# tub-rip/MotionPriorCMax

Measured on AMD Instinct MI355X. Metric: Mevents/s through CMax loss fwd+bwd, DSEC 480x640, higher is better.
Workload: dtype f32; 1 GPU; C3: DSEC 480x640, 200k events/window, poly-k3, batch=14 per GPU (BASELINE configs[2]; the per-GPU shard of configs[4] = batch 112 on 8 GPUs); batch_per_gpu=14, events_layout=time, resident_batches_rotated=4, global_batch=14, num_bins=15, num_knn=32, parallelism=dp1, grad_allreduce_MB=0

## Files before the change

### motionpriorcmax_amd/csrc/diag/stamps.h

```cpp
#pragma once

#ifdef KNN_BK_STAMP
#define BK_STAMP_DECL __shared__ unsigned s_stp[8];
#define BK_STAMP(k) do { __builtin_amdgcn_s_waitcnt(0); if (threadIdx.x == 0) s_stp[k] = (unsigned)wall_clock64(); } while (0)
#define BK_STAMP_WRITE(ls_, tid_) do { BK_STAMP(7); __syncthreads(); \
        if ((tid_) < 8) (ls_).fail[1 + 100000 + 8 * blockIdx.x + (tid_)] = (tid_) == 0 ? (int)s_stp[0] : (int)(s_stp[tid_] - s_stp[0]); } while (0)
#else
#define BK_STAMP_DECL
#define BK_STAMP(k) do { } while (0)
#define BK_STAMP_WRITE(ls_, tid_) do { } while (0)
#endif

#if defined(KS_STAMP2) || defined(KS_STAMP0)
#ifdef KS_STAMP0
#define KS_STP_ON (MODE == 0)
#else
#define KS_STP_ON (FARK)
#endif
#define KS_STP_DECL unsigned long long stp_[8]; int nstp_ = 0;
#define KS_STP() do { if (KS_STP_ON && nstp_ < 8) { __builtin_amdgcn_s_waitcnt(0); stp_[nstp_++] = wall_clock64(); } } while (0)
#define KS_STP_WRITE(ls_, tid_, mine_, total_) do { if (KS_STP_ON) { __syncthreads(); KS_STP(); const int nmk_ = __syncthreads_count((mine_) ? 1 : 0); \
        if ((tid_) == 0) { int *dst_ = (ls_).fail + 1 + 200000 + 12 * (int)blockIdx.x; dst_[0] = (int)(stp_[0] & 0x7fffffffull); \
            for (int k_ = 1; k_ < 8; ++k_) dst_[k_] = (int)(stp_[k_] - stp_[0]); dst_[8] = (total_); dst_[9] = nmk_; } } } while (0)
#else
#define KS_STP_DECL
#define KS_STP() do { } while (0)
#define KS_STP_WRITE(ls_, tid_, mine_, total_) do { } while (0)
#endif

#ifdef KS_DEBUG_INBIN
#define KS_INBIN_STAT(knn_state_, BQ_, q_, inbin_, nsl_, iwd_, norm_) do { (knn_state_)[2 * (BQ_) + (q_)] = (float)(inbin_) + 100.f * (float)(nsl_); } while (0)
#else
#define KS_INBIN_STAT(knn_state_, BQ_, q_, inbin_, nsl_, iwd_, norm_) do { if (iwd_) (knn_state_)[2 * (BQ_) + (q_)] = (norm_); } while (0)
#endif

#ifdef KNN_BW_STAMP
#define KB_STAMP_PARAM , int *__restrict__ stamp
#define KB_STAMP_BEGIN const unsigned long long st0 = wall_clock64(); int st_slow = 0;
#define KB_STAMP_MID const unsigned long long st1 = wall_clock64();
#define KB_STAMP_SLOW st_slow = 1;
#define KB_STAMP_END(tid_, lblk_, RQ_, use_lds_, anytie_, total_) do { __syncthreads(); const bool anyslow_ = __syncthreads_or(st_slow) != 0; \
        if ((tid_) == 0) { const unsigned long long st2_ = wall_clock64(); stamp[4 * (lblk_) + 0] = (int)(st2_ - st0); stamp[4 * (lblk_) + 1] = (int)(st1 - st0); \
            stamp[4 * (lblk_) + 2] = (RQ_) | ((use_lds_) ? 0 : 256) | ((anytie_) ? 512 : 0) | (anyslow_ ? 1024 : 0); stamp[4 * (lblk_) + 3] = (total_); } } while (0)
#define KB_STAMP_ARG(ws_, L_) , (int *)((char *)(ws_) + (L_).off_knn_fail)
#else
#define KB_STAMP_PARAM
#define KB_STAMP_BEGIN
#define KB_STAMP_MID
#define KB_STAMP_SLOW
#define KB_STAMP_END(tid_, lblk_, RQ_, use_lds_, anytie_, total_) do { } while (0)
#define KB_STAMP_ARG(ws_, L_)
#endif

#ifdef EV_LA_STAMP
#define LA_STAMP_DECL __shared__ unsigned s_stp[8]; if (threadIdx.x < 8) s_stp[threadIdx.x] = (unsigned)wall_clock64();
#define LA_STAMP(k) do { __builtin_amdgcn_s_waitcnt(0); if (threadIdx.x == 0) s_stp[k] = (unsigned)wall_clock64(); } while (0)
#define LA_STAMP_WRITE(tid_, dst_, n_) do { LA_STAMP(6); __syncthreads(); if ((tid_) == 0) { unsigned *d_ = reinterpret_cast<unsigned *>(dst_); \
        for (int k_ = 0; k_ < 7; ++k_) d_[k_] = s_stp[k_] - s_stp[0]; d_[7] = (unsigned)(n_); d_[8] = s_stp[0]; } } while (0)
#else
#define LA_STAMP_DECL
#define LA_STAMP(k) do { } while (0)
#define LA_STAMP_WRITE(tid_, dst_, n_) do { } while (0)
#endif

#ifdef KT_TIMELINE
#define KT_T(k_) do { __builtin_amdgcn_s_waitcnt(0); if (threadIdx.x == 0) kt_[k_] = (int)(wall_clock64() & 0x7fffffffull); } while (0)
#define KT_DECL int kt_[6] = {0, 0, 0, 0, 0, 0};
#define KT_COUNT(k_, n_) do { kt_[k_] = (n_); } while (0)
#define KT_WRITE(ls_) do { if (threadIdx.x == 0) { int *d_ = (ls_).fail + 1 + 300000 + 8 * (int)blockIdx.x; for (int k_ = 0; k_ < 6; ++k_) d_[k_] = kt_[k_]; } } while (0)
#else
#define KT_T(k_) do { } while (0)
#define KT_DECL
#define KT_COUNT(k_, n_) do { } while (0)
#define KT_WRITE(ls_) do { } while (0)
#endif
```

### motionpriorcmax_amd/csrc/events.hip

```cpp
#include "common.h"
#include "ev_count_device.h"
#include "knn_device.h"
#include "bounds.h"
#include "diag/stamps.h"

struct EvParams {
    int B, M, Mp, nb, T, H, W, sp, hq, wq, P;
    unsigned flags;
};

struct Warped {
    float y, x, w;
    int lut;
    float fy, fx;
    int y0, x0;
    int it, iy, ix;
};

__device__ __forceinline__ EvParams make_params(const mpc_shape s) {
    EvParams p;
    p.B = s.B; p.M = s.M; p.Mp = s.Mp; p.nb = s.nb; p.T = s.T; p.H = s.H; p.W = s.W;
    p.sp = s.sp; p.hq = s.hq; p.wq = s.wq;
    p.P = (s.flags & MPC_F_POLARITY_SPLIT) ? 2 : 1;
    p.flags = s.flags;
// ... 22 lines not shown
        const float dt = fminf(fmaxf(fabsf(e[2] - t_ref), 0.f), 1.f);
        w = (1.f - dt) * w;
    }
    if (p.flags & MPC_F_MASK_BORDER) {
        if (y > (float)p.H || x > (float)p.W || y < 0.f || x < 0.f) w = 0.f;
    }
    o.y = y; o.x = x; o.w = w;
    const float y0f = floorf(y + 1e-6f), x0f = floorf(x + 1e-6f);
    o.fy = y - y0f;
    o.fx = x - x0f;
    o.y0 = (int)fminf(fmaxf(y0f, -4.f), (float)p.H + 4.f);
    o.x0 = (int)fminf(fmaxf(x0f, -4.f), (float)p.W + 4.f);
    return w != 0.f;
}

__device__ __forceinline__ bool warp_event(const EvParams &p, const float e[6], int b, int tr,
                                           const float *__restrict__ lut, float t_ref, Warped &o) {
    o.lut = -1;
    float2 f = make_float2(0.f, 0.f);
    if (!(p.flags & MPC_F_NO_WARP)) {
        warp_cell(p, e, b, tr, o);
        f = reinterpret_cast<const float2 *>(lut)[o.lut];
    }
    return warp_event_with(p, e, f, t_ref, o);
}

__device__ __forceinline__ void load_event(const float *__restrict__ events, size_t row, float e[6]) {
    const float2 *p = reinterpret_cast<const float2 *>(events + row * 6);
    const float2 a = p[0], b = p[1], c = p[2];
    e[0] = a.x; e[1] = a.y; e[2] = b.x; e[3] = b.y; e[4] = c.x; e[5] = c.y;
}

__global__ __launch_bounds__(256) void k_splat_fwd_atomic(const mpc_shape s,
                                                          const float *__restrict__ events,
                                                          const float *__restrict__ lut,
                                                          const float *__restrict__ t_ref,
                                                          float *__restrict__ iwe) {
    const EvParams p = make_params(s);
    const size_t total = (size_t)p.B * p.M;
    for (size_t row = (size_t)blockIdx.x * 256 + threadIdx.x; row < total; row += (size_t)gridDim.x * 256) {
        const int b = (int)(row / p.M), i = (int)(row - (size_t)b * p.M);
        float e[6];
        load_event(events, row, e);
        const int pol = (p.P == 2 && i >= p.Mp) ? 1 : 0;
        for (int tr = 0; tr < p.T; ++tr) {
            Warped o;
            const float tref = (p.flags & MPC_F_SCALE_BY_DT) ? t_ref[tr] : 0.f;
            if (!warp_event(p, e, b, tr, lut, tref, o)) continue;
            float *img = iwe + ((size_t)(b * p.T + tr) * p.P + pol) * p.H * p.W;
            const float w00 = (1.f - o.fy) * (1.f - o.fx) * o.w;
            const float w10 = o.fy * (1.f - o.fx) * o.w;
            const float w01 = (1.f - o.fy) * o.fx * o.w;
            const float w11 = o.fy * o.fx * o.w;
            const bool yin0 = o.y0 >= 0 && o.y0 < p.H, yin1 = o.y0 + 1 >= 0 && o.y0 + 1 < p.H;
            const bool xin0 = o.x0 >= 0 && o.x0 < p.W, xin1 = o.x0 + 1 >= 0 && o.x0 + 1 < p.W;
            if (yin0 && xin0) atomicAdd(img + (size_t)o.y0 * p.W + o.x0, w00);
            if (yin1 && xin0) atomicAdd(img + (size_t)(o.y0 + 1) * p.W + o.x0, w10);
            if (yin0 && xin1) atomicAdd(img + (size_t)o.y0 * p.W + o.x0 + 1, w01);
            if (yin1 && xin1) atomicAdd(img + (size_t)(o.y0 + 1) * p.W + o.x0 + 1, w11);
        }
    }
}

__device__ __forceinline__ void event_pos_grad(const EvParams &p, const Warped &o,
                                               const float *__restrict__ g , float &gy,
                                               float &gx) {
    const bool yin0 = o.y0 >= 0 && o.y0 < p.H, yin1 = o.y0 + 1 >= 0 && o.y0 + 1 < p.H;
    const bool xin0 = o.x0 >= 0 && o.x0 < p.W, xin1 = o.x0 + 1 >= 0 && o.x0 + 1 < p.W;
    const float g00 = (yin0 && xin0) ? g[(size_t)o.y0 * p.W + o.x0] : 0.f;
    const float g10 = (yin1 && xin0) ? g[(size_t)(o.y0 + 1) * p.W + o.x0] : 0.f;
    const float g01 = (yin0 && xin1) ? g[(size_t)o.y0 * p.W + o.x0 + 1] : 0.f;
    const float g11 = (yin1 && xin1) ? g[(size_t)(o.y0 + 1) * p.W + o.x0 + 1] : 0.f;
    gy = o.w * ((1.f - o.fx) * (g10 - g00) + o.fx * (g11 - g01));
    gx = o.w * ((1.f - o.fy) * (g01 - g00) + o.fy * (g11 - g10));
}

__global__ __launch_bounds__(256) void k_splat_bwd_atomic(const mpc_shape s,
                                                          const float *__restrict__ events,
                                                          const float *__restrict__ lut,
                                                          const float *__restrict__ t_ref,
                                                          const float *__restrict__ gimg,
                                                          const float *__restrict__ scal,
                                                          const float *__restrict__ grad_out,
                                                          float *__restrict__ glut) {
    const EvParams p = make_params(s);
    const float coef = scal[MPC_SCAL_GCOEF] * (grad_out ? grad_out[0] : 1.f);
    const size_t total = (size_t)p.B * p.M;
    for (size_t row = (size_t)blockIdx.x * 256 + threadIdx.x; row < total; row += (size_t)gridDim.x * 256) {
        const int b = (int)(row / p.M), i = (int)(row - (size_t)b * p.M);
        float e[6];
        load_event(events, row, e);
        const int pol = (p.P == 2 && i >= p.Mp) ? 1 : 0;
        for (int tr = 0; tr < p.T; ++tr) {
            Warped o;
            const float tref = (p.flags & MPC_F_SCALE_BY_DT) ? t_ref[tr] : 0.f;
            if (!warp_event(p, e, b, tr, lut, tref, o)) continue;
            const float *img = gimg + ((size_t)(b * p.T + tr) * p.P + pol) * p.H * p.W;
            float gy, gx;
            event_pos_grad(p, o, img, gy, gx);
            atomicAdd(glut + 2 * (size_t)o.lut, coef * gy);
            atomicAdd(glut + 2 * (size_t)o.lut + 1, coef * gx);
        }
    }
}

__global__ __launch_bounds__(256) void k_event_pos_grad(const mpc_shape s, const float *__restrict__ events,
                                                        const float *__restrict__ t_ref, const float *__restrict__ gimg,
                                                        const float *__restrict__ scal, const float *__restrict__ grad_out,
                                                        float2 *__restrict__ gpos) {
    const EvParams p = make_params(s);
    const float coef = scal[MPC_SCAL_GCOEF] * (grad_out ? grad_out[0] : 1.f);
    const float tref = (p.flags & MPC_F_SCALE_BY_DT) ? t_ref[0] : 0.f;
    const size_t total = (size_t)p.B * p.M;
    for (size_t row = (size_t)blockIdx.x * 256 + threadIdx.x; row < total; row += (size_t)gridDim.x * 256) {
        const int b = (int)(row / p.M), i = (int)(row - (size_t)b * p.M);
        float e[6];
        load_event(events, row, e);
        const int pol = (p.P == 2 && i >= p.Mp) ? 1 : 0;
        Warped o;
        float2 g = make_float2(0.f, 0.f);
        if (warp_event_with(p, e, make_float2(0.f, 0.f), tref, o)) {
            float gy, gx;
            event_pos_grad(p, o, gimg + ((size_t)b * p.P + pol) * p.H * p.W, gy, gx);
            g = make_float2(coef * gy, coef * gx);
        }
        gpos[row] = g;
    }
}

#define EV_MARKER 0x6d706331

struct BinLayout {
    int SR, NS, CSR, NCS, NF, NBk, fcap, bcap, P, exact;
    int *gcount;
    int *bcapcnt;
    float4 *frec, *brec;
};

struct __attribute__((packed, aligned(4))) rec3 { float y, x, w; };

__device__ __forceinline__ long long ev_to_fixed_small(float v) {
    return (long long)(int)(v * (float)(1 << MPC_FIX_SHIFT));
}

__device__ __forceinline__ int xcd_swizzle(int p, int n) {
    const int per = (n + 7) >> 3;
    return (p & 7) * per + (p >> 3);
}


__device__ __forceinline__ void ev_emit(const EvParams &p, const BinLayout &L, int b, int nf_loc, int lb, int slot,
                                        float4 rec) {
    if (lb < nf_loc) {
        const int g = (b * p.P + lb / L.NS) * L.NS + (lb % L.NS);
        MPC_EXPECT(g >= 0 && g < L.NF);
        reinterpret_cast<rec3 *>(L.frec)[(size_t)g * L.fcap + MPC_IDX(slot, L.fcap)] = rec3{rec.x, rec.y, rec.z};
    } else {
        const size_t base = L.exact ? (size_t)b : (size_t)(b * p.nb * L.NCS + (lb - nf_loc));
        MPC_EXPECT((long long)base < (L.exact ? (long long)p.B : (long long)L.NBk));
        L.brec[base * L.bcap + MPC_IDX(slot, L.bcap)] = rec;
    }
}

__global__ __launch_bounds__(256) void k_ev_bin(const mpc_shape s, const BinLayout L,
                                                const float *__restrict__ events,
                                                const float *__restrict__ lut,
                                                const float *__restrict__ t_ref, int want_bwd,
                                                const int *__restrict__ offsets) {
    extern __shared__ __align__(16) int s_cnt[];
    __shared__ int s_wsum[4];
    const EvParams p = make_params(s);
    const int chunks = (p.M + 256 * EV_PER_THREAD - 1) / (256 * EV_PER_THREAD);
    const int lblk = xcd_swizzle(blockIdx.x, chunks * p.B);
    if (lblk >= chunks * p.B) return;
    const int tid = threadIdx.x, b = lblk / chunks, chunk = lblk - b * chunks;
    int pad0 = p.M, pad1 = p.M, blk1 = p.M;
    if (offsets != nullptr) {
        const int nk1 = p.nb * L.NCS + 1;
        const int *ob = offsets + (size_t)b * 2 * nk1;
        blk1 = p.Mp;
        pad0 = min(max(ob[nk1 - 1], 0), blk1);
        pad1 = min(max(ob[2 * nk1 - 1], blk1), p.M);
        const int c0 = chunk * EV_PER_THREAD * 256, c1 = min(c0 + EV_PER_THREAD * 256, p.M);
        const bool all_pad = (c0 >= pad0 && c1 <= blk1) || c0 >= pad1;
        if (all_pad) return;
    }
    const int nf_loc = p.P * L.NS, nb_loc = want_bwd ? p.nb * L.NCS : 0, nloc = nf_loc + nb_loc;
    int *s_base = s_cnt + nloc;
    const int stage_off = ((3 * nloc + 1 + EV_STAGE / 2) + 3) & ~3;
    for (int i = tid; i < nloc; i += 256) s_cnt[i] = 0;
    __syncthreads();
    const float tref = (p.flags & MPC_F_SCALE_BY_DT) ? t_ref[0] : 0.f;
    const float inv_SR = 1.f / (float)L.SR, inv_CSR = 1.f / (float)L.CSR;

    float ry[EV_PER_THREAD], rx[EV_PER_THREAD], rw[EV_PER_THREAD];
    int f0[EV_PER_THREAD], f1[EV_PER_THREAD], bk[EV_PER_THREAD];
    int r0[EV_PER_THREAD], r1[EV_PER_THREAD], rb[EV_PER_THREAD];
    unsigned aux[EV_PER_THREAD];
    float ev[EV_PER_THREAD][6];
    Warped wo[EV_PER_THREAD];
    bool live[EV_PER_THREAD];
#pragma unroll
    for (int k = 0; k < EV_PER_THREAD; ++k) {
        const int i = (chunk * EV_PER_THREAD + k) * 256 + tid;
        load_event(events, (size_t)b * p.M + min(i, p.M - 1), ev[k]);
    }
#pragma unroll
    for (int k = 0; k < EV_PER_THREAD; ++k) {
        const int i = (chunk * EV_PER_THREAD + k) * 256 + tid;
        live[k] = warp_event(p, ev[k], b, 0, lut, tref, wo[k]) && (i < p.M) && !((i >= pad0 && i < blk1) || i >= pad1);
    }
#pragma unroll
    for (int k = 0; k < EV_PER_THREAD; ++k) {
        const int i = (chunk * EV_PER_THREAD + k) * 256 + tid;
        f0[k] = f1[k] = bk[k] = -1;
        r0[k] = r1[k] = rb[k] = 0;
        ry[k] = rx[k] = rw[k] = 0.f; aux[k] = 0u;
        if (!live[k]) continue;
        const Warped &o = wo[k];
        const bool xin = (o.x0 + 1 >= 0) && (o.x0 < p.W);
        const bool yin0 = o.y0 >= 0 && o.y0 < p.H, yin1 = o.y0 + 1 >= 0 && o.y0 + 1 < p.H;
        if (!xin || !(yin0 || yin1)) continue;
        const int pol = (p.P == 2 && i >= p.Mp) ? 1 : 0;
        ry[k] = o.y; rx[k] = o.x; rw[k] = o.w;
        const int s0 = yin0 ? (int)(((float)o.y0 + 0.5f) * inv_SR) : -1, s1 = yin1 ? (int)(((float)o.y0 + 1.5f) * inv_SR) : -1;
        if (s0 >= 0) { f0[k] = pol * L.NS + s0; r0[k] = atomicAdd(&s_cnt[MPC_IDX(f0[k], nf_loc)], 1); }
        if (s1 >= 0 && s1 != s0) { f1[k] = pol * L.NS + s1; r1[k] = atomicAdd(&s_cnt[MPC_IDX(f1[k], nf_loc)], 1); }
        if (want_bwd && o.lut >= 0) {
            const int cst = (int)(((float)o.iy + 0.5f) * inv_CSR);
            bk[k] = nf_loc + o.it * L.NCS + cst;
            rb[k] = atomicAdd(&s_cnt[MPC_IDX(bk[k], nloc)], 1);
            aux[k] = ((unsigned)pol << 31) | (unsigned)((o.iy - cst * L.CSR) * p.wq + o.ix);
        }
    }
    __syncthreads();
    for (int i = tid; i < nloc; i += 256) {
        const int c = s_cnt[i];
        int g;
        int first = 0;
        if (i < nf_loc) g = (b * p.P + i / L.NS) * L.NS + (i % L.NS);
        else { g = L.NF + b * p.nb * L.NCS + (i - nf_loc); if (L.exact) first = L.bcapcnt[L.NBk + b * p.nb * L.NCS + (i - nf_loc)]; }
        s_base[i] = (c > 0 ? atomicAdd(&L.gcount[MPC_IDX(g, L.NF + L.NBk)], c) : 0) + first;
    }
    int *s_loc = s_base + nloc;
    unsigned short *s_bid = reinterpret_cast<unsigned short *>(s_loc + nloc + 1);
    float4 *s_rec = reinterpret_cast<float4 *>(s_cnt + stage_off);
    {
        const int per = (nloc + 255) >> 8;
        const int i0 = min(tid * per, nloc), i1 = min(i0 + per, nloc);
        int local = 0;
        for (int i = i0; i < i1; ++i) local += s_cnt[i];
        int incl = local;
#pragma unroll
        for (int o = 1; o < 64; o <<= 1) { const int v = __shfl_up(incl, o, 64); if ((tid & 63) >= o) incl += v; }
        if ((tid & 63) == 63) s_wsum[tid >> 6] = incl;
        __syncthreads();
        int run = incl - local;
        for (int w = 0; w < (tid >> 6); ++w) run += s_wsum[w];
        for (int i = i0; i < i1; ++i) { s_loc[i] = run; run += s_cnt[i]; }
        if (tid == 255) s_loc[nloc] = run;
    }
    __syncthreads();
    const int total = s_loc[nloc];
#pragma unroll
    for (int k = 0; k < EV_PER_THREAD; ++k) {
        if (f0[k] >= 0 || f1[k] >= 0) {
            const int polf = (f0[k] >= 0 ? f0[k] : f1[k]) / L.NS;
            const float4 rec = make_float4(ry[k], rx[k], rw[k], __int_as_float(b * p.P + polf));
#pragma unroll
            for (int h = 0; h < 2; ++h) {
                const int lb = h ? f1[k] : f0[k];
                if (lb < 0) continue;
                const int at = s_loc[lb] + (h ? r1[k] : r0[k]);
                if (at < EV_STAGE) { s_rec[MPC_IDX(at, EV_STAGE)] = rec; s_bid[MPC_IDX(at, EV_STAGE)] = (unsigned short)lb; }
                else ev_emit(p, L, b, nf_loc, lb, s_base[lb] + (h ? r1[k] : r0[k]), rec);
            }
        }
        if (bk[k] >= 0) {
            const float4 rec = make_float4(ry[k], rx[k], rw[k], __uint_as_float(aux[k]));
            const int at = s_loc[bk[k]] + rb[k];
            if (at < EV_STAGE) { s_rec[MPC_IDX(at, EV_STAGE)] = rec; s_bid[MPC_IDX(at, EV_STAGE)] = (unsigned short)bk[k]; }
            else ev_emit(p, L, b, nf_loc, bk[k], s_base[bk[k]] + rb[k], rec);
        }
    }
    __syncthreads();
    for (int r = tid; r < min(total, EV_STAGE); r += 256) {
        const int lb = s_bid[r];
        ev_emit(p, L, b, nf_loc, lb, s_base[MPC_IDX(lb, nloc)] + (r - s_loc[lb]), s_rec[r]);
    }
    if (want_bwd && lblk == 0 && tid == 0) L.gcount[L.NF + L.NBk + 2] = EV_MARKER;
}

template <typename F>
__device__ __forceinline__ void record_taps(float y, float x, float w, int H, int W, int row0, int row1, F f) {
    const float y0f = floorf(y + 1e-6f), x0f = floorf(x + 1e-6f);
    const float fy = y - y0f, fx = x - x0f;
    const int y0 = (int)fminf(fmaxf(y0f, -4.f), (float)H + 4.f), x0 = (int)fminf(fmaxf(x0f, -4.f), (float)W + 4.f);
    const bool r0 = y0 >= row0 && y0 < row1, r1 = y0 + 1 >= row0 && y0 + 1 < row1;
    const bool c0 = x0 >= 0 && x0 < W, c1 = x0 + 1 >= 0 && x0 + 1 < W;
    if (r0 && c0) f(y0, x0, (1.f - fy) * (1.f - fx) * w);
    if (r1 && c0) f(y0 + 1, x0, fy * (1.f - fx) * w);
    if (r0 && c1) f(y0, x0 + 1, (1.f - fy) * fx * w);
    if (r1 && c1) f(y0 + 1, x0 + 1, fy * fx * w);
}

template <bool FIXED>
__global__ __launch_bounds__(1024) void k_iwe_accum(const BinLayout L, float *__restrict__ iwe, int H, int W) {
    extern __shared__ unsigned long long s_acc[];
    const int tid = threadIdx.x;
    const int g = blockIdx.x, img = g / L.NS, strip = g - img * L.NS;
    const int row0 = strip * L.SR, row1 = min(row0 + L.SR, H);
    const int npix = (row1 - row0) * W;
    const int n = L.gcount[g];
    const rec3 *rec = reinterpret_cast<const rec3 *>(L.frec) + (size_t)g * L.fcap;
    rec3 e[4];
#pragma unroll
    for (int u = 0; u < 4; ++u) e[u] = rec[MPC_IDX(min(tid + u * 1024, L.fcap - 1), L.fcap)];
    for (int i = tid; i < npix; i += 1024) s_acc[i] = 0ull;
    __syncthreads();
    for (int r0 = tid; r0 < n; r0 += 4 * 1024) {
        if (r0 != tid) {
#pragma unroll
            for (int u = 0; u < 4; ++u) e[u] = rec[min(r0 + u * 1024, n - 1)];
        }
#pragma unroll
        for (int u = 0; u < 4; ++u) {
            if (r0 + u * 1024 >= n) continue;
            if (fabsf(e[u].w) <= 1.5f)
                record_taps(e[u].y, e[u].x, e[u].w, H, W, row0, row1, [&](int yy, int xx, float v) {
                    atomicAdd(&s_acc[MPC_IDX((yy - row0) * W + xx, npix)], (unsigned long long)ev_to_fixed_small(v));
                });
            else
                record_taps(e[u].y, e[u].x, e[u].w, H, W, row0, row1, [&](int yy, int xx, float v) {
                    atomicAdd(&s_acc[MPC_IDX((yy - row0) * W + xx, npix)], (unsigned long long)mpc_to_fixed(v));
                });
        }
    }
    __syncthreads();
    if (FIXED) {
        long long *dst = reinterpret_cast<long long *>(iwe) + ((size_t)img * H + row0) * W;
        for (int i = tid; i < npix; i += 1024) dst[i] = (long long)s_acc[i];
    } else {
        float *dst = iwe + ((size_t)img * H + row0) * W;
        for (int i = tid; i < npix; i += 1024) dst[i] = mpc_from_fixed((long long)s_acc[i]);
    }
}

__global__ __launch_bounds__(256) void k_iwe_from_fixed(const long long *__restrict__ src, float *__restrict__ dst, size_t n) {
    for (size_t i = (size_t)blockIdx.x * 256 + threadIdx.x; i < n; i += (size_t)gridDim.x * 256) dst[i] = mpc_from_fixed(src[i]);
}

struct __attribute__((packed, aligned(4))) pair4 { float x, y; };

__device__ __forceinline__ void record_grad(float y, float x, float w, const float *__restrict__ g, int H, int W,
                                            float &gy, float &gx) {
    const float y0f = floorf(y + 1e-6f), x0f = floorf(x + 1e-6f);
    const float fy = y - y0f, fx = x - x0f;
    const int y0 = (int)fminf(fmaxf(y0f, -4.f), (float)H + 4.f), x0 = (int)fminf(fmaxf(x0f, -4.f), (float)W + 4.f);
    const bool r0 = y0 >= 0 && y0 < H, r1 = y0 + 1 >= 0 && y0 + 1 < H;
    const bool c0 = x0 >= 0 && x0 < W, c1 = x0 + 1 >= 0 && x0 + 1 < W;
    const int xa = min(max(x0, 0), W - 2);
    const int ya = min(max(y0, 0), H - 1), yb = min(max(y0 + 1, 0), H - 1);
    const pair4 a = *reinterpret_cast<const pair4 *>(g + MPC_IDX((size_t)ya * W + xa, (long long)H * W - 1));
    const pair4 b = *reinterpret_cast<const pair4 *>(g + MPC_IDX((size_t)yb * W + xa, (long long)H * W - 1));
    const bool lo = (xa == x0);
    const float g00 = (r0 && c0) ? (lo ? a.x : a.y) : 0.f;
    const float g01 = (r0 && c1) ? (lo ? a.y : a.x) : 0.f;
    const float g10 = (r1 && c0) ? (lo ? b.x : b.y) : 0.f;
    const float g11 = (r1 && c1) ? (lo ? b.y : b.x) : 0.f;
    gy = w * ((1.f - fx) * (g10 - g00) + fx * (g11 - g01));
    gx = w * ((1.f - fy) * (g01 - g00) + fy * (g11 - g10));
}

template <bool ORDERED>
__global__ __launch_bounds__(ORDERED ? EV_LUT_THREADS_ORD : EV_LUT_THREADS, ORDERED ? 1 : EV_LUT_MINWAVES) void k_lut_accum(const mpc_shape s, const BinLayout L,
                                                    const float *__restrict__ gimg,
                                                    const float *__restrict__ scal,
                                                    const float *__restrict__ grad_out,
                                                    float *__restrict__ glut,
                                                    const float *__restrict__ add_term,
                                                    const float *__restrict__ events, const float *__restrict__ lut,
                                                    const float *__restrict__ t_ref, const int *__restrict__ offsets,
                                                    const KnnReachJob job) {
    extern __shared__ unsigned long long s_acc[];
    LA_STAMP_DECL
    constexpr int NT = ORDERED ? EV_LUT_THREADS_ORD : EV_LUT_THREADS, NIF = ORDERED ? EV_LUT_INFLIGHT_ORD : EV_LUT_INFLIGHT;
    constexpr int APF = ORDERED ? 0 : EV_LUT_ADD_PF;
    const EvParams p = make_params(s);
    const int tid = threadIdx.x;
    const int lg = xcd_swizzle(blockIdx.x, L.NBk);
    if (lg >= L.NBk) return;
    const int b = lg / (L.NCS * p.nb), rem = lg - b * (L.NCS * p.nb);
    const int cst = rem / p.nb, it = rem - cst * p.nb;
    const int bt = b * p.nb + it;
    const int g = bt * L.NCS + cst;
    const int crow0 = cst * L.CSR, crow1 = min(crow0 + L.CSR, p.hq);
    const int ncell = (crow1 - crow0) * p.wq;
    const int NK = p.nb * L.NCS, key = it * L.NCS + cst;
    float4 e[NIF];
    float2 addv[APF > 0 ? APF : 1];
    int mark = 0, n = 0;
    float gcoef = 0.f, gout = 1.f;
    const float4 *rec = L.brec;
    int rcap = L.bcap;
    const float2 *add = add_term ? reinterpret_cast<const float2 *>(add_term) + ((size_t)bt * p.hq + crow0) * p.wq : nullptr;
    const bool spec = !ORDERED && !(p.flags & MPC_F_NO_BWD_RECORDS);
    if (!ORDERED) {
        mark = L.gcount[L.NF + L.NBk + 2];
        n = L.gcount[L.NF + g];
        int first = 0;
        if (L.exact) first = min(max(L.bcapcnt[L.NBk + (size_t)b * NK + key], 0), L.bcap - 1);
        rec = L.brec + (size_t)(L.exact ? b : g) * L.bcap + first;
        rcap = L.bcap - first;
        const float4 *src = spec ? rec : reinterpret_cast<const float4 *>(L.gcount);
        const int last = spec ? rcap - 1 : 0;
#pragma unroll
        for (int u = 0; u < NIF; ++u) e[u] = src[MPC_IDX(min(tid + u * NT, last), last + 1)];
        gcoef = scal[MPC_SCAL_GCOEF];
        if (grad_out) gout = grad_out[0];
        if (add && ncell > 0) {
#pragma unroll
            for (int k = 0; k < APF; ++k) addv[k] = add[MPC_IDX(min(tid + k * NT, ncell - 1), ncell)];
        }
    }
    if (job.on && cst == 0) {
        if (job.p.l1) knn_reach_slice<true>(job.p, job.tile_dkmax, job.reach, bt, job.gx, job.gy, job.bd, reinterpret_cast<float *>(s_acc));
        else knn_reach_slice<false>(job.p, job.tile_dkmax, job.reach, bt, job.gx, job.gy, job.bd, reinterpret_cast<float *>(s_acc));
        __syncthreads();
    }
    for (int i = tid; i < 2 * ncell; i += NT) s_acc[i] = 0ull;
    float2 *s_lut = reinterpret_cast<float2 *>(s_acc + 2 * ncell);
    if (ORDERED) {
        const float2 *src = reinterpret_cast<const float2 *>(lut) + ((size_t)(b * p.nb + it) * p.hq + crow0) * p.wq;
        for (int i = tid; i < ncell; i += NT) s_lut[i] = src[i];
    }
    __syncthreads();
    LA_STAMP(1);
    const bool valid = ORDERED || mark == EV_MARKER;
    int n_pos = 0, o_pos = 0, o_neg = 0;
    if (ORDERED) {
        const int *ob = offsets + (size_t)b * 2 * (NK + 1);
        o_pos = min(max(ob[key], 0), p.M); n_pos = min(max(ob[key + 1] - o_pos, 0), p.M - o_pos);
// ... 7 lines not shown
        const int pol = r >= n_pos ? 1 : 0;
        const int row = pol ? o_neg + (r - n_pos) : o_pos + r;
        float e[6];
        load_event(events, (size_t)b * p.M + row, e);
        Warped o;
        warp_cell(p, e, b, 0, o);
        const bool here = o.it == it && o.iy >= crow0 && o.iy < crow1;
        const int cell = here ? (o.iy - crow0) * p.wq + o.ix : 0;
        const bool mine = warp_event_with(p, e, s_lut[MPC_IDX(cell, ncell)], tref, o) && here;
        const unsigned aux = ((unsigned)((p.P == 2) ? pol : 0) << 31) | (unsigned)cell;
        return make_float4(o.y, o.x, mine ? o.w : 0.f, __uint_as_float(aux));
    };
    for (int r0 = tid; r0 < n; r0 += NIF * NT) {
        if (spec && r0 == tid) {
#pragma unroll
            for (int u = 0; u < NIF; ++u) if (r0 + u * NT >= n) e[u] = make_float4(0.f, 0.f, 0.f, 0.f);
        } else {
#pragma unroll
            for (int u = 0; u < NIF; ++u) e[u] = fetch(min(r0 + u * NT, n - 1));
        }
        LA_STAMP(3);
        float gy[NIF], gx[NIF];
#pragma unroll
        for (int u = 0; u < NIF; ++u) {
            const int pol = (int)(__float_as_uint(e[u].w) >> 31);
            record_grad(e[u].x, e[u].y, e[u].z, gimg + (size_t)(b * p.P + pol) * p.H * p.W, p.H, p.W, gy[u], gx[u]);
        }
        LA_STAMP(4);
#pragma unroll
        for (int u = 0; u < NIF; ++u) {
            if (r0 + u * NT < n && (!ORDERED || e[u].z != 0.f)) {
                const int cell = (int)(__float_as_uint(e[u].w) & 0x7fffffffu);
                atomicAdd(&s_acc[MPC_IDX(2 * cell, 2 * ncell)], (unsigned long long)mpc_to_fixed(gy[u]));
                atomicAdd(&s_acc[MPC_IDX(2 * cell + 1, 2 * ncell)], (unsigned long long)mpc_to_fixed(gx[u]));
            }
        }
    }
    __syncthreads();
    LA_STAMP(5);
    if (ORDERED) { gout = grad_out ? grad_out[0] : 1.f; gcoef = scal[MPC_SCAL_GCOEF]; }
    const float coef = valid ? gcoef * gout : __int_as_float(0x7fc00000);
    float2 *dst = reinterpret_cast<float2 *>(glut) + ((size_t)bt * p.hq + crow0) * p.wq;
    auto put = [&](int i, bool have, float2 o) {
        float2 v = make_float2(coef * mpc_from_fixed((long long)s_acc[2 * i]), coef * mpc_from_fixed((long long)s_acc[2 * i + 1]));
        if (add) { if (!have) o = add[i]; v.x += gout * o.x; v.y += gout * o.y; }
        dst[i] = v;
    };
#pragma unroll
    for (int k = 0; k < APF; ++k) if (tid + k * NT < ncell) put(tid + k * NT, true, addv[k]);
    for (int i = tid + APF * NT; i < ncell; i += NT) put(i, false, make_float2(0.f, 0.f));
    LA_STAMP_WRITE(tid, dst, n);
}

__global__ __launch_bounds__(256) void k_ev_count(const EvCountArgs a) {
    extern __shared__ int s_ec[];
    ev_count_block(a, blockIdx.x, s_ec);
}
__global__ __launch_bounds__(256) void k_ev_prefix(const EvCountArgs a) {
    __shared__ int s_tmp[4];
    ev_prefix_block(a, blockIdx.x, s_tmp);
}

static BinLayout bin_layout(const mpc_shape *s, const mpc_ws_layout &L, void *ws) {
    BinLayout B;
    B.SR = L.strip_rows; B.NS = L.n_strips; B.CSR = L.cstrip_rows; B.NCS = L.n_cstrips;
    B.NF = L.nfb; B.NBk = L.nbb; B.fcap = L.fcap; B.bcap = L.bcap; B.P = L.P; B.exact = L.b_exact;
    B.gcount = (int *)((char *)ws + L.off_fcount);
    B.bcapcnt = B.gcount + L.nfb + L.nbb + 8;
    B.frec = (float4 *)((char *)ws + L.off_frec);
    B.brec = (float4 *)((char *)ws + L.off_brec);
    return B;
}

EvCountArgs mpc_event_count_args(const mpc_shape *s, const float *events, void *ws) {
    EvCountArgs a{};
    const mpc_ws_layout L = mpc_layout(s);
    const bool tiled = !(s->flags & MPC_F_ATOMIC_PATH) && s->T == 1 && L.strip_rows > 0 && L.cstrip_rows > 0;
    if (!tiled || !L.b_exact || (s->flags & (MPC_F_NO_WARP | MPC_F_NO_BWD_RECORDS)) || s->B <= 0 || s->M <= 0 || !events) return a;
    a.events = events;
    a.cap = (int *)((char *)ws + L.off_fcount) + L.nfb + L.nbb + 8;
    a.B = s->B; a.M = s->M; a.nb = s->nb; a.sp = s->sp; a.hq = s->hq; a.CSR = L.cstrip_rows; a.NCS = L.n_cstrips;
    return a;
}

static bool use_tiled(const mpc_shape *s, const mpc_ws_layout &L) { return !(s->flags & MPC_F_ATOMIC_PATH) && s->T == 1 && L.strip_rows > 0 && L.cstrip_rows > 0; }

static int set_max_lds_ev(const void *fn, const char *who) {
    hipError_t e = hipFuncSetAttribute(fn, hipFuncAttributeMaxDynamicSharedMemorySize, 160 * 1024 - 512);
    if (e != hipSuccess) { mpc_set_error("%s: %s", who, hipGetErrorString(e)); return (int)e; }
    return 0;
}

extern "C" int mpc_event_splat_fwd(const mpc_shape *s, const float *events, const float *flow_lut,
                                   const float *t_ref, float *iwe_raw, void *ws, void *stream) {
    return mpc_event_splat_fwd_ex(s, events, flow_lut, t_ref, iwe_raw, ws, stream, 0, nullptr);
}

static int splat_fwd_impl(const mpc_shape *s, const float *events, const float *flow_lut, const float *t_ref,
                          float *iwe_raw, void *ws, void *stream, int counters_zeroed, bool fixed, const int32_t *offsets = nullptr);

extern "C" int mpc_event_splat_fwd_fixed(const mpc_shape *s, const float *events, const float *flow_lut, const float *t_ref,
                                         int64_t *iwe_fixed, void *ws, void *stream) {
    MPC_CHECK_ARG(s && iwe_fixed && ws, MPC_E_NULL, "null argument");
    MPC_CHECK_ARG(!(s->flags & MPC_F_ATOMIC_PATH) && s->T == 1, MPC_E_UNSUPPORTED, "fixed-point images come from the LDS-tiled path (num_tref == 1)");
    return splat_fwd_impl(s, events, flow_lut, t_ref, reinterpret_cast<float *>(iwe_fixed), ws, stream, 0, true);
}

extern "C" int mpc_iwe_from_fixed(const int64_t *iwe_fixed, float *iwe_raw, int64_t count, void *stream) {
    MPC_CHECK_ARG((iwe_fixed && iwe_raw) || count == 0, MPC_E_NULL, "null argument");
    if (count <= 0) return 0;
    const int64_t blocks = (count + 255) / 256 < 8192 ? (count + 255) / 256 : 8192;
    MPC_LAUNCH(k_iwe_from_fixed, dim3((unsigned)blocks), dim3(256), 0, (hipStream_t)stream, reinterpret_cast<const long long *>(iwe_fixed), iwe_raw, (size_t)count);
    MPC_CHECK_LAUNCH();
    return 0;
}

int mpc_event_splat_fwd_ex(const mpc_shape *s, const float *events, const float *flow_lut, const float *t_ref,
                           float *iwe_raw, void *ws, void *stream, int counters_zeroed, const int32_t *offsets) {
    return splat_fwd_impl(s, events, flow_lut, t_ref, iwe_raw, ws, stream, counters_zeroed, false, offsets);
}

static int splat_fwd_impl(const mpc_shape *s, const float *events, const float *flow_lut, const float *t_ref,
                          float *iwe_raw, void *ws, void *stream, int counters_zeroed, bool fixed, const int32_t *offsets) {
    MPC_CHECK_ARG(s && iwe_raw && ws && (events || s->M == 0 || s->B == 0), MPC_E_NULL, "null argument");
    MPC_CHECK_ARG((s->flags & MPC_F_NO_WARP) || flow_lut, MPC_E_NULL, "flow_lut is null");
    MPC_CHECK_ARG(!(s->flags & MPC_F_SCALE_BY_DT) || t_ref, MPC_E_NULL, "t_ref is null");
    int rc = mpc_validate_shape(s);
    if (rc) return rc;
    const mpc_ws_layout L = mpc_layout(s);
    hipStream_t st = (hipStream_t)stream;
    if (use_tiled(s, L)) {
        static mpc_device_once attr_once;
        if (attr_once.need()) {
            if ((rc = set_max_lds_ev((const void *)k_iwe_accum<false>, __func__))) return rc;
            if ((rc = set_max_lds_ev((const void *)k_iwe_accum<true>, __func__))) return rc;
            if ((rc = set_max_lds_ev((const void *)k_lut_accum<false>, __func__))) return rc;
            if ((rc = set_max_lds_ev((const void *)k_lut_accum<true>, __func__))) return rc;
            attr_once.mark();
        }
        const BinLayout BL = bin_layout(s, L, ws);
        const int want_bwd = (s->flags & (MPC_F_NO_WARP | MPC_F_NO_BWD_RECORDS)) ? 0 : 1;
        if (!(counters_zeroed & 1) && (rc = mpc_zero_async(BL.gcount, (size_t)(L.nfb + 2 * L.nbb + 8) * sizeof(int), st))) return rc;
        if (s->B > 0 && s->M > 0) {
            const int nblk = mpc_cdiv(s->M, 256 * EV_PER_THREAD) * s->B;
            const dim3 grid(((nblk + 7) / 8) * 8);
            if (want_bwd && L.b_exact && !(counters_zeroed & 2)) {
                const EvCountArgs ca = mpc_event_count_args(s, events, ws);
                MPC_LAUNCH(k_ev_count, dim3(ev_count_blocks(ca)), dim3(256), (size_t)s->nb * L.n_cstrips * sizeof(int), st, ca);
                MPC_LAUNCH(k_ev_prefix, dim3(s->B), dim3(256), 0, st, ca);
                MPC_CHECK_LAUNCH();
            }
            const int nloc = L.P * L.n_strips + s->nb * L.n_cstrips;
            const size_t lds = (size_t)(((3 * nloc + 1 + EV_STAGE / 2) + 3) & ~3) * sizeof(int) + (size_t)EV_STAGE * 16;
            MPC_LAUNCH(k_ev_bin, grid, dim3(256), lds, st, *s, BL, events, flow_lut, t_ref, want_bwd, want_bwd ? nullptr : offsets);
            MPC_CHECK_LAUNCH();
        }
        if (L.nfb > 0) {
            if (fixed) MPC_LAUNCH(k_iwe_accum<true>, dim3(L.nfb), dim3(1024), (size_t)L.strip_rows * s->W * 8, st, BL, iwe_raw, s->H, s->W);
            else MPC_LAUNCH(k_iwe_accum<false>, dim3(L.nfb), dim3(1024), (size_t)L.strip_rows * s->W * 8, st, BL, iwe_raw, s->H, s->W);
            MPC_CHECK_LAUNCH();
        }
        return 0;
    }
    MPC_CHECK_ARG(!fixed, MPC_E_UNSUPPORTED, "fixed-point images need the LDS-tiled path");
    const size_t img_bytes = (size_t)L.nimg * s->H * s->W * sizeof(float);
    const int e = mpc_zero_async(iwe_raw, img_bytes, st);
    if (e) return e;
    const int64_t total = (int64_t)s->B * s->M;
    if (total == 0) return 0;
    const int grid = (int)((total + 255) / 256 < 8192 ? (total + 255) / 256 : 8192);
    MPC_LAUNCH(k_splat_fwd_atomic, dim3(grid), dim3(256), 0, st, *s, events, flow_lut, t_ref, iwe_raw);
    MPC_CHECK_LAUNCH();
    return 0;
}

extern "C" int mpc_event_splat_bwd(const mpc_shape *s, const float *events, const float *flow_lut,
                                   const float *t_ref, const float *grad_iwe, const float *scal,
                                   const float *grad_out, float *grad_flow_lut, const float *add_term,
                                   void *ws, void *stream) {
    return mpc_event_splat_bwd_ordered(s, events, nullptr, flow_lut, t_ref, grad_iwe, scal, grad_out, grad_flow_lut, add_term, ws, stream);
}

extern "C" int mpc_event_splat_bwd_ordered(const mpc_shape *s, const float *events, const int32_t *offsets, const float *flow_lut,
                                           const float *t_ref, const float *grad_iwe, const float *scal,
                                           const float *grad_out, float *grad_flow_lut, const float *add_term,
                                           void *ws, void *stream) {
    return mpc_event_splat_bwd_job(s, events, offsets, flow_lut, t_ref, grad_iwe, scal, grad_out, grad_flow_lut, add_term, ws, stream, nullptr, nullptr);
}

int mpc_event_splat_bwd_job(const mpc_shape *s, const float *events, const int32_t *offsets, const float *flow_lut,
                            const float *t_ref, const float *grad_iwe, const float *scal,
                            const float *grad_out, float *grad_flow_lut, const float *add_term,
                            void *ws, void *stream, const float *knn_state, int *reach_done) {
    if (reach_done) *reach_done = 0;
    MPC_CHECK_ARG(s && flow_lut && grad_iwe && scal && grad_flow_lut && ws && (events || s->M == 0 || s->B == 0), MPC_E_NULL, "null argument");
    MPC_CHECK_ARG(!(s->flags & MPC_F_NO_WARP), MPC_E_UNSUPPORTED, "no LUT to differentiate with MPC_F_NO_WARP");
    MPC_CHECK_ARG(!(s->flags & MPC_F_SCALE_BY_DT) || t_ref, MPC_E_NULL, "t_ref is null");
    int rc = mpc_validate_shape(s);
    if (rc) return rc;
    hipStream_t st = (hipStream_t)stream;
    const mpc_ws_layout L = mpc_layout(s);
    if (use_tiled(s, L)) {
        const BinLayout BL = bin_layout(s, L, ws);
        if (L.nbb > 0) {
            MPC_CHECK_ARG(!offsets || (size_t)L.cstrip_rows * s->wq * 24 <= 160 * 1024 - 512, MPC_E_UNSUPPORTED,
                          "LUT too wide for the ordered backward (use mpc_event_splat_bwd)");
            KnnReachJob job{};
            const size_t lds_acc = (size_t)L.cstrip_rows * s->wq * (offsets ? 24 : 16);
            if (knn_state && mpc_knn_reach_job(s, knn_state, ws, &job) &&
                ((size_t)job.gx * job.gy * (KNN_NCLS + 1) + 16) * sizeof(float) > lds_acc) job.on = 0;
            if (offsets)
                MPC_LAUNCH(k_lut_accum<true>, dim3(((L.nbb + 7) / 8) * 8), dim3(EV_LUT_THREADS_ORD), lds_acc, st, *s, BL,
                                   grad_iwe, scal, grad_out, grad_flow_lut, add_term, events, flow_lut, t_ref, offsets, job);
            else
                MPC_LAUNCH(k_lut_accum<false>, dim3(((L.nbb + 7) / 8) * 8), dim3(EV_LUT_THREADS), lds_acc, st, *s, BL,
                                   grad_iwe, scal, grad_out, grad_flow_lut, add_term, events, flow_lut, t_ref, offsets, job);
            MPC_CHECK_LAUNCH();
            if (reach_done) *reach_done = job.on;
        }
        return 0;
    }
    {
        const int64_t cnt = (int64_t)s->B * s->nb * s->hq * s->wq * s->T * 2;
        if (add_term) {
            rc = grad_out ? mpc_scale(add_term, grad_out, grad_flow_lut, cnt, stream) : (int)hipMemcpyAsync(grad_flow_lut, add_term, cnt * sizeof(float), hipMemcpyDeviceToDevice, st);
            if (rc) return rc;
        } else {
            const int e = mpc_zero_async(grad_flow_lut, cnt * sizeof(float), st);
            if (e) return e;
        }
    }
    const int64_t total = (int64_t)s->B * s->M;
    if (total == 0) return 0;
    const int grid = (int)((total + 255) / 256 < 8192 ? (total + 255) / 256 : 8192);
    MPC_LAUNCH(k_splat_bwd_atomic, dim3(grid), dim3(256), 0, st, *s, events, flow_lut, t_ref,
                       grad_iwe, scal, grad_out, grad_flow_lut);
    MPC_CHECK_LAUNCH();
    return 0;
}


#define PE_KMAX 8
template <int KB>
__device__ __forceinline__ void pe_phi(const float *__restrict__ phi, size_t row, int k, float t, float tref, float *out ) {
    const int kk = KB > 0 ? KB : min(k, PE_KMAX);
    if (phi != nullptr) { for (int j = 0; j < kk; ++j) out[j] = phi[row * k + j]; return; }
    float a = tref, c = t;
    for (int j = 0; j < kk; ++j) { out[j] = a - c; a *= tref; c *= t; }
}

template <int KB>
__global__ __launch_bounds__(256) void k_pe_warp(const mpc_shape s, const float *__restrict__ events, const float *__restrict__ coef,
                                                 const float *__restrict__ phi, int k, const float *__restrict__ t_ref,
                                                 float *__restrict__ rows_out) {
    const EvParams p = make_params(s);
    const float tref = t_ref ? t_ref[0] : 0.f;
    const size_t total = (size_t)p.B * p.M;
    for (size_t row = (size_t)blockIdx.x * 256 + threadIdx.x; row < total; row += (size_t)gridDim.x * 256) {
        const int b = (int)(row / p.M);
        float e[6];
        load_event(events, row, e);
        const int iy = min(max((int)floorf(mpc_div_sp(e[0], p.sp)), 0), p.hq - 1), ix = min(max((int)floorf(mpc_div_sp(e[1], p.sp)), 0), p.wq - 1);
        const int cell = (b * p.hq + iy) * p.wq + ix;
        const float *c = coef + (size_t)cell * 2 * k;
        float fy = 0.f, fx = 0.f;
        float ph[KB > 0 ? KB : PE_KMAX];
        pe_phi<KB>(phi, row, k, e[2], tref, ph);
        if (KB > 0) {
#pragma unroll
            for (int j = 0; j < KB; ++j) { fy += c[j] * ph[j]; fx += c[KB + j] * ph[j]; }
        } else {
            for (int j = 0; j < k; ++j) { const float f = j < PE_KMAX ? ph[j] : phi[row * k + j]; fy += c[j] * f; fx += c[k + j] * f; }
        }
        float2 *o = reinterpret_cast<float2 *>(rows_out + row * 6);
        o[0] = make_float2(e[0] + fy, e[1] + fx);
        o[1] = make_float2(e[2], e[3]);
        o[2] = make_float2(__int_as_float(cell), e[5]);
    }
}

template <int KB>
__global__ __launch_bounds__(256) void k_pe_grad(const mpc_shape s, const float *__restrict__ rows, const float *__restrict__ phi, int k,
                                                 const float *__restrict__ t_ref, const float *__restrict__ gimg,
                                                 const float *__restrict__ scal, const float *__restrict__ grad_out,
                                                 float *__restrict__ gcoef) {
    const EvParams p = make_params(s);
    const float coef = scal[MPC_SCAL_GCOEF] * (grad_out ? grad_out[0] : 1.f);
    const float tref = t_ref[0];
    const size_t total = (size_t)p.B * p.M;
    for (size_t row = (size_t)blockIdx.x * 256 + threadIdx.x; row < total; row += (size_t)gridDim.x * 256) {
        const int b = (int)(row / p.M), i = (int)(row - (size_t)b * p.M);
        float e[6];
        load_event(rows, row, e);
        const int pol = (p.P == 2 && i >= p.Mp) ? 1 : 0;
        Warped o;
        if (!warp_event_with(p, e, make_float2(0.f, 0.f), tref, o)) continue;
        float gy, gx;
        event_pos_grad(p, o, gimg + ((size_t)b * p.P + pol) * p.H * p.W, gy, gx);
        gy *= coef; gx *= coef;
        if (gy == 0.f && gx == 0.f) continue;
        const int cell = __float_as_int(e[4]);
        float *g = gcoef + (size_t)cell * 2 * k;
        const int kk = KB > 0 ? KB : k;
        float ph[KB > 0 ? KB : PE_KMAX];
        pe_phi<KB>(phi, row, k, e[2], tref, ph);
        for (int j = 0; j < kk; ++j) { const float f = j < PE_KMAX ? ph[j] : phi[row * k + j]; atomicAdd(g + j, f * gy); atomicAdd(g + kk + j, f * gx); }
    }
// ... 324 lines not shown
```

Baseline: 4856 Mevents/s.

## Overlap bucket-base atomics with LDS staging in event binning kernel

After: 4854 Mevents/s. Within noise of the previous version (-0.0%).

```diff
diff --git a/motionpriorcmax_amd/csrc/diag/stamps.h b/motionpriorcmax_amd/csrc/diag/stamps.h
--- a/motionpriorcmax_amd/csrc/diag/stamps.h
+++ b/motionpriorcmax_amd/csrc/diag/stamps.h
@@ -63,6 +63,23 @@
 #define LA_STAMP_WRITE(tid_, dst_, n_) do { } while (0)
 #endif
 
+#ifdef EV_BIN_STAMP
+#define EB_STAMP_PARAM , int *__restrict__ stamp
+#define EB_STAMP_ARG(ws_, L_) , (int *)((char *)(ws_) + (L_).off_knn_fail) + 1 + 400000
+#define EB_STAMP_DECL __shared__ unsigned s_ebs[8]; if (threadIdx.x < 8) s_ebs[threadIdx.x] = (unsigned)wall_clock64();
+#define EB_STAMP(k) do { __builtin_amdgcn_s_waitcnt(0); if (threadIdx.x == 0) s_ebs[k] = (unsigned)wall_clock64(); } while (0)
+#define EB_STAMP_LDS(k) do { __builtin_amdgcn_s_waitcnt(0xc07f); if (threadIdx.x == 0) s_ebs[k] = (unsigned)wall_clock64(); } while (0)
+#define EB_STAMP_WRITE(tid_, lblk_) do { EB_STAMP(6); __syncthreads(); if ((tid_) < 8) \
+        stamp[8 * (lblk_) + (tid_)] = (tid_) == 0 ? 0 : (tid_) == 7 ? (int)(s_ebs[0] & 0x7fffffffu) : (int)(s_ebs[tid_] - s_ebs[0]); } while (0)
+#else
+#define EB_STAMP_PARAM
+#define EB_STAMP_ARG(ws_, L_)
+#define EB_STAMP_DECL
+#define EB_STAMP(k) do { } while (0)
+#define EB_STAMP_LDS(k) do { } while (0)
+#define EB_STAMP_WRITE(tid_, lblk_) do { } while (0)
+#endif
+
 #ifdef KT_TIMELINE
 #define KT_T(k_) do { __builtin_amdgcn_s_waitcnt(0); if (threadIdx.x == 0) kt_[k_] = (int)(wall_clock64() & 0x7fffffffull); } while (0)
 #define KT_DECL int kt_[6] = {0, 0, 0, 0, 0, 0};
diff --git a/motionpriorcmax_amd/csrc/events.hip b/motionpriorcmax_amd/csrc/events.hip
--- a/motionpriorcmax_amd/csrc/events.hip
+++ b/motionpriorcmax_amd/csrc/events.hip
@@ -198,8 +198,8 @@
 __device__ __forceinline__ void ev_emit(const EvParams &p, const BinLayout &L, int b, int nf_loc, int lb, int slot,
                                         float4 rec) {
     if (lb < nf_loc) {
-        const int g = (b * p.P + lb / L.NS) * L.NS + (lb % L.NS);
-        MPC_EXPECT(g >= 0 && g < L.NF);
+        const int g = b * nf_loc + lb;
+        MPC_EXPECT(g >= 0 && g < L.NF && nf_loc == p.P * L.NS);
         reinterpret_cast<rec3 *>(L.frec)[(size_t)g * L.fcap + MPC_IDX(slot, L.fcap)] = rec3{rec.x, rec.y, rec.z};
     } else {
         const size_t base = L.exact ? (size_t)b : (size_t)(b * p.nb * L.NCS + (lb - nf_loc));
@@ -208,11 +208,28 @@
     }
 }
 
+__device__ __forceinline__ int ev_global_bucket(const EvParams &p, const BinLayout &L, int b, int nf_loc, int i) {
+    return i < nf_loc ? b * nf_loc + i : L.NF + b * p.nb * L.NCS + (i - nf_loc);
+}
+__device__ __forceinline__ int ev_first_load(const EvParams &p, const BinLayout &L, int b, int nf_loc, int nloc, int i) {
+    if (!L.exact) return 0;
+    return L.bcapcnt[MPC_IDX(L.NBk + b * p.nb * L.NCS + ((i >= nf_loc && i < nloc) ? i - nf_loc : 0), 2 * L.NBk)];
+}
+__device__ __forceinline__ int ev_first_of(int loaded, int nf_loc, int i) { return i >= nf_loc ? loaded : 0; }
+
+__device__ __forceinline__ void ev_lds_barrier() {
+    __builtin_amdgcn_fence(__ATOMIC_RELEASE, "workgroup", "local");
+    __builtin_amdgcn_s_barrier();
+    __builtin_amdgcn_fence(__ATOMIC_ACQUIRE, "workgroup", "local");
+}
+
+#define EV_BIN_REG 2
+
 __global__ __launch_bounds__(256) void k_ev_bin(const mpc_shape s, const BinLayout L,
                                                 const float *__restrict__ events,
                                                 const float *__restrict__ lut,
                                                 const float *__restrict__ t_ref, int want_bwd,
-                                                const int *__restrict__ offsets) {
+                                                const int *__restrict__ offsets EB_STAMP_PARAM) {
     extern __shared__ __align__(16) int s_cnt[];
     __shared__ int s_wsum[4];
     const EvParams p = make_params(s);
@@ -234,6 +251,11 @@
     const int nf_loc = p.P * L.NS, nb_loc = want_bwd ? p.nb * L.NCS : 0, nloc = nf_loc + nb_loc;
     int *s_base = s_cnt + nloc;
     const int stage_off = ((3 * nloc + 1 + EV_STAGE / 2) + 3) & ~3;
+    EB_STAMP_DECL
+    const bool base_in_regs = nloc <= 256 * EV_BIN_REG;
+    int afirst[EV_BIN_REG];
+#pragma unroll
+    for (int u = 0; u < EV_BIN_REG; ++u) afirst[u] = (base_in_regs && want_bwd) ? ev_first_load(p, L, b, nf_loc, nloc, tid + 256 * u) : 0;
     for (int i = tid; i < nloc; i += 256) s_cnt[i] = 0;
     __syncthreads();
     const float tref = (p.flags & MPC_F_SCALE_BY_DT) ? t_ref[0] : 0.f;
@@ -256,6 +278,7 @@
         const int i = (chunk * EV_PER_THREAD + k) * 256 + tid;
         live[k] = warp_event(p, ev[k], b, 0, lut, tref, wo[k]) && (i < p.M) && !((i >= pad0 && i < blk1) || i >= pad1);
     }
+    EB_STAMP(1);
 #pragma unroll
     for (int k = 0; k < EV_PER_THREAD; ++k) {
         const int i = (chunk * EV_PER_THREAD + k) * 256 + tid;
@@ -280,14 +303,24 @@
         }
     }
     __syncthreads();
-    for (int i = tid; i < nloc; i += 256) {
-        const int c = s_cnt[i];
-        int g;
-        int first = 0;
-        if (i < nf_loc) g = (b * p.P + i / L.NS) * L.NS + (i % L.NS);
-        else { g = L.NF + b * p.nb * L.NCS + (i - nf_loc); if (L.exact) first = L.bcapcnt[L.NBk + b * p.nb * L.NCS + (i - nf_loc)]; }
-        s_base[i] = (c > 0 ? atomicAdd(&L.gcount[MPC_IDX(g, L.NF + L.NBk)], c) : 0) + first;
-    }
+    EB_STAMP_LDS(2);
+    int araw[EV_BIN_REG];
+    if (base_in_regs) {
+        int c[EV_BIN_REG];
+#pragma unroll
+        for (int u = 0; u < EV_BIN_REG; ++u) c[u] = tid + 256 * u < nloc ? s_cnt[tid + 256 * u] : 0;
+#pragma unroll
+        for (int u = 0; u < EV_BIN_REG; ++u) {
+            araw[u] = 0;
+            if (c[u] > 0) araw[u] = atomicAdd(&L.gcount[MPC_IDX(ev_global_bucket(p, L, b, nf_loc, tid + 256 * u), L.NF + L.NBk)], c[u]);
+        }
+    } else {
+        for (int i = tid; i < nloc; i += 256) {
+            const int c = s_cnt[i];
+            s_base[i] = (c > 0 ? atomicAdd(&L.gcount[MPC_IDX(ev_global_bucket(p, L, b, nf_loc, i), L.NF + L.NBk)], c) : 0) + ev_first_of(ev_first_load(p, L, b, nf_loc, nloc, i), nf_loc, i);
+        }
+    }
+    EB_STAMP_LDS(3);
     int *s_loc = s_base + nloc;
     unsigned short *s_bid = reinterpret_cast<unsigned short *>(s_loc + nloc + 1);
     float4 *s_rec = reinterpret_cast<float4 *>(s_cnt + stage_off);
@@ -300,40 +333,54 @@
 #pragma unroll
         for (int o = 1; o < 64; o <<= 1) { const int v = __shfl_up(incl, o, 64); if ((tid & 63) >= o) incl += v; }
         if ((tid & 63) == 63) s_wsum[tid >> 6] = incl;
-        __syncthreads();
+        ev_lds_barrier();
         int run = incl - local;
         for (int w = 0; w < (tid >> 6); ++w) run += s_wsum[w];
         for (int i = i0; i < i1; ++i) { s_loc[i] = run; run += s_cnt[i]; }
         if (tid == 255) s_loc[nloc] = run;
     }
-    __syncthreads();
+    ev_lds_barrier();
+    EB_STAMP_LDS(4);
     const int total = s_loc[nloc];
-#pragma unroll
-    for (int k = 0; k < EV_PER_THREAD; ++k) {
-        if (f0[k] >= 0 || f1[k] >= 0) {
-            const int polf = (f0[k] >= 0 ? f0[k] : f1[k]) / L.NS;
-            const float4 rec = make_float4(ry[k], rx[k], rw[k], __int_as_float(b * p.P + polf));
-#pragma unroll
-            for (int h = 0; h < 2; ++h) {
-                const int lb = h ? f1[k] : f0[k];
-                if (lb < 0) continue;
-                const int at = s_loc[lb] + (h ? r1[k] : r0[k]);
-                if (at < EV_STAGE) { s_rec[MPC_IDX(at, EV_STAGE)] = rec; s_bid[MPC_IDX(at, EV_STAGE)] = (unsigned short)lb; }
-                else ev_emit(p, L, b, nf_loc, lb, s_base[lb] + (h ? r1[k] : r0[k]), rec);
+    auto walk = [&](const bool over) {
+#pragma unroll
+        for (int k = 0; k < EV_PER_THREAD; ++k) {
+            if (f0[k] >= 0 || f1[k] >= 0) {
+                const int polf = (f0[k] >= 0 ? f0[k] : f1[k]) >= L.NS ? 1 : 0;
+                const float4 rec = make_float4(ry[k], rx[k], rw[k], __int_as_float(b * p.P + polf));
+#pragma unroll
+                for (int h = 0; h < 2; ++h) {
+                    const int lb = h ? f1[k] : f0[k];
+                    if (lb < 0) continue;
+                    const int at = s_loc[lb] + (h ? r1[k] : r0[k]);
+                    if (!over) { if (at < EV_STAGE) { s_rec[MPC_IDX(at, EV_STAGE)] = rec; s_bid[MPC_IDX(at, EV_STAGE)] = (unsigned short)lb; } }
+                    else if (at >= EV_STAGE) ev_emit(p, L, b, nf_loc, lb, s_base[MPC_IDX(lb, nloc)] + (h ? r1[k] : r0[k]), rec);
+                }
             }
-        }
-        if (bk[k] >= 0) {
-            const float4 rec = make_float4(ry[k], rx[k], rw[k], __uint_as_float(aux[k]));
-            const int at = s_loc[bk[k]] + rb[k];
-            if (at < EV_STAGE) { s_rec[MPC_IDX(at, EV_STAGE)] = rec; s_bid[MPC_IDX(at, EV_STAGE)] = (unsigned short)bk[k]; }
-            else ev_emit(p, L, b, nf_loc, bk[k], s_base[bk[k]] + rb[k], rec);
-        }
-    }
-    __syncthreads();
+            if (bk[k] >= 0) {
+                const float4 rec = make_float4(ry[k], rx[k], rw[k], __uint_as_float(aux[k]));
+                const int at = s_loc[bk[k]] + rb[k];
+                if (!over) { if (at < EV_STAGE) { s_rec[MPC_IDX(at, EV_STAGE)] = rec; s_bid[MPC_IDX(at, EV_STAGE)] = (unsigned short)bk[k]; } }
+                else if (at >= EV_STAGE) ev_emit(p, L, b, nf_loc, bk[k], s_base[MPC_IDX(bk[k], nloc)] + rb[k], rec);
+            }
+        }
+    };
+    walk(false);
+    if (base_in_regs) {
+#pragma unroll
+        for (int u = 0; u < EV_BIN_REG; ++u) {
+            const int i = tid + 256 * u;
+            if (i < nloc) s_base[i] = araw[u] + ev_first_of(afirst[u], nf_loc, i);
+        }
+    }
+    ev_lds_barrier();
+    EB_STAMP_LDS(5);
     for (int r = tid; r < min(total, EV_STAGE); r += 256) {
         const int lb = s_bid[r];
         ev_emit(p, L, b, nf_loc, lb, s_base[MPC_IDX(lb, nloc)] + (r - s_loc[lb]), s_rec[r]);
     }
+    if (total > EV_STAGE) walk(true);
+    EB_STAMP_WRITE(tid, lblk);
     if (want_bwd && lblk == 0 && tid == 0) L.gcount[L.NF + L.NBk + 2] = EV_MARKER;
 }
 
@@ -647,7 +694,7 @@
             }
             const int nloc = L.P * L.n_strips + s->nb * L.n_cstrips;
             const size_t lds = (size_t)(((3 * nloc + 1 + EV_STAGE / 2) + 3) & ~3) * sizeof(int) + (size_t)EV_STAGE * 16;
-            MPC_LAUNCH(k_ev_bin, grid, dim3(256), lds, st, *s, BL, events, flow_lut, t_ref, want_bwd, want_bwd ? nullptr : offsets);
+            MPC_LAUNCH(k_ev_bin, grid, dim3(256), lds, st, *s, BL, events, flow_lut, t_ref, want_bwd, want_bwd ? nullptr : offsets EB_STAMP_ARG(ws, L));
             MPC_CHECK_LAUNCH();
         }
         if (L.nfb > 0) {
```
